# jhamrick/bayesian-quadrature

Hardware: AMD Instinct MI355X
Metric: bq_fit_posterior_throughput (higher is better)
Workload: dtype f64; 1 GPU; C2: d=1 N=1024 M=256 Gaussian integrand, w=dx, s=1e-3; curve_workload=C5 shard: 64 x (d=1 N=2048 M=256), w=dx, s=1e-2, on_curve=True, bordered_system=1344

## Files before the change

### bayesian-quadrature_amd/csrc/ctx.hip

```cpp
#include "host.h"

namespace bqh {

int prof_collect(bq_ctx *c)
{
    if (c->prof_events.empty())
        return BQ_OK;
    HIPCHK(c, hipStreamSynchronize(c->stream));
    if (c->aux)
        HIPCHK(c, hipStreamSynchronize(c->aux));
    if (c->prof_keep_timeline && !c->prof_origin)
        c->prof_origin = c->prof_events.front().a;
    for (auto &e : c->prof_events) {
        float ms = 0.f;
        if (hipEventElapsedTime(&ms, e.a, e.b) == hipSuccess) {
            c->prof_ms[e.cls] += ms;
            c->prof_n[e.cls] += 1;
            c->prof_work[e.cls] += e.work;
            if (c->prof_keep_timeline) {
                float t0 = 0.f;
                (void)hipEventElapsedTime(&t0, c->prof_origin, e.a);
                c->prof_timeline.insert(c->prof_timeline.end(),
                                        {(double)e.cls, (double)e.on_aux, (double)t0,
                                         (double)t0 + ms, e.work});
            }
        }
    }
    for (auto &e : c->prof_events) {
        if (e.a != c->prof_origin)
            (void)hipEventDestroy(e.a);
        (void)hipEventDestroy(e.b);
    }
    c->prof_events.clear();
    return BQ_OK;
}

int check_dims(bq_ctx *c, int64_t d, int64_t n)
{
    if (!c)
        return BQ_ERR_BAD_ARG;
    if (d < 1 || d > BQ_MAXD)
        return fail(c, BQ_ERR_BAD_ARG, "d must be in 1..%d", BQ_MAXD);
    if (n < 1 || n > (1 << 20))
        return fail(c, BQ_ERR_BAD_ARG, "n out of range");
    return BQ_OK;
}

int check_w(bq_ctx *c, int64_t d, double h, const double *w, double s)
{
    if (!w)
        return fail(c, BQ_ERR_BAD_ARG, "w is NULL");
    if (!(std::isfinite(h)) || !(std::isfinite(s)))
        return fail(c, BQ_ERR_BAD_ARG, "h and s must be finite");
    for (int k = 0; k < d; ++k)
        if (!(w[k] > 0.0) || !std::isfinite(w[k]))
            return fail(c, BQ_ERR_BAD_ARG, "w must be positive and finite");
    return BQ_OK;
}


}

using namespace bqh;

extern "C" int bq_device_count(int *count)
{
    if (!count)
        return BQ_ERR_BAD_ARG;
    int n = 0;
    if (hipGetDeviceCount(&n) != hipSuccess)
        n = 0;
    *count = n;
    return BQ_OK;
}

static int ctx_init(bq_ctx *c, int device)
{
    HIPCHK(c, hipSetDevice(device));
    c->device = device;
    hipDeviceProp_t prop;
    HIPCHK(c, hipGetDeviceProperties(&prop, device));
    c->cus = prop.multiProcessorCount > 0 ? prop.multiProcessorCount : 256;
    HIPCHK(c, hipEventCreate(&c->t0));
    HIPCHK(c, hipEventCreate(&c->t1));
    HIPCHK(c, hipEventCreateWithFlags(&c->ev_panel, hipEventDisableTiming));
    HIPCHK(c, hipEventCreateWithFlags(&c->ev_next, hipEventDisableTiming));
    HIPCHK(c, hipEventCreateWithFlags(&c->ev_fork, hipEventDisableTiming));
    HIPCHK(c, hipEventCreateWithFlags(&c->ev_top, hipEventDisableTiming));

    int lo = 0, hi = 0;
    HIPCHK(c, hipDeviceGetStreamPriorityRange(&lo, &hi));
    HIPCHK(c, hipStreamCreateWithPriority(&c->aux, hipStreamNonBlocking, hi));
    BQCHK(gemm_init(c));
    {
        void *h = nullptr;
        HIPCHK(c, hipHostMalloc(&h, 64, hipHostMallocMapped));
        c->flow_abort = static_cast<int *>(h);
        *c->flow_abort = 0;
    }
    static const struct {
        const char *name;
        int bq_ctx::*field;
    } switches[] = {
        {"BQ_TRSV_FLOW", &bq_ctx::trsv_flow},
        {"BQ_LOOKAHEAD", &bq_ctx::lookahead},
        {"BQ_DIAG_FIRST", &bq_ctx::diag_first},
        {"BQ_ASM_FUSE", &bq_ctx::asm_fuse},
        {"BQ_DF_SWEEP", &bq_ctx::df_sweep},
        {"BQ_DF_WG", &bq_ctx::df_wg},
        {"BQ_PAIR_BORDER", &bq_ctx::pair_border},
        {"BQ_DF_WG_ROWS", &bq_ctx::df_wg_rows},
        {"BQ_DF_EARLY", &bq_ctx::df_early},
        {"BQ_SOLVE_KCOPY", &bq_ctx::solve_kcopy},
        {"BQ_LA_MIN", &bq_ctx::la_min},
        {"BQ_GEMM_LDS", &bq_ctx::gemm_lds},
        {"BQ_FOLD_READOUT", &bq_ctx::fold_readout},
        {"BQ_POTF2_8W", &bq_ctx::potf2_8w},
        {"BQ_GEMM_KSPLIT", &bq_ctx::gemm_ksplit},
        {"BQ_GEMM_TILE", &bq_ctx::gemm_tile},
        {"BQ_GRAPH", &bq_ctx::use_graph},
    };
    for (const auto &sw : switches)
        if (const char *e = std::getenv(sw.name))
            c->*sw.field = std::atoi(e);
    return BQ_OK;
}

extern "C" int bq_ctx_create(int device, bq_ctx **out)
{
    if (!out)
        return BQ_ERR_BAD_ARG;
    *out = nullptr;
    bq_ctx *c = new (std::nothrow) bq_ctx();
    if (!c)
        return BQ_ERR_NOMEM;
    int st = ctx_init(c, device);
    if (st == BQ_OK) {
        hipError_t e = hipStreamCreateWithFlags(&c->stream, hipStreamNonBlocking);
        if (e != hipSuccess)
            st = fail(c, BQ_ERR_HIP, "hipStreamCreate: %s", hipGetErrorString(e));
        c->own_stream = true;
        c->cur = c->stream;
    }
    if (st != BQ_OK) {
        fprintf(stderr, "bq_ctx_create: %s\n", c->err);
        delete c;
        return st;
    }
    *out = c;
    return BQ_OK;
}

extern "C" int bq_ctx_create_on_stream(int device, void *hip_stream, bq_ctx **out)
{
    if (!out)
        return BQ_ERR_BAD_ARG;
    *out = nullptr;
    bq_ctx *c = new (std::nothrow) bq_ctx();
    if (!c)
        return BQ_ERR_NOMEM;
    int st = ctx_init(c, device);
    if (st != BQ_OK) {
        delete c;
        return st;
    }
    c->stream = static_cast<hipStream_t>(hip_stream);
    c->cur = c->stream;
    c->own_stream = false;
    *out = c;
    return BQ_OK;
}

extern "C" void bq_ctx_destroy(bq_ctx *c)
{
    if (!c)
        return;
    (void)hipSetDevice(c->device);
    (void)hipStreamSynchronize(c->stream);
    if (c->plan_cache) {
        bq_plan_destroy(c, c->plan_cache);
        c->plan_cache = nullptr;
    }
    for (auto &e : c->prof_events) {
        if (e.a != c->prof_origin)
            (void)hipEventDestroy(e.a);
        (void)hipEventDestroy(e.b);
    }
    if (c->prof_origin)
        (void)hipEventDestroy(c->prof_origin);
    if (c->t0)
        (void)hipEventDestroy(c->t0);
    if (c->t1)
        (void)hipEventDestroy(c->t1);
    if (c->hstage)
        (void)hipHostFree(c->hstage);
    c->hstage = nullptr;
    for (hipEvent_t e : {c->ev_panel, c->ev_next, c->ev_fork, c->ev_top})
        if (e)
            (void)hipEventDestroy(e);
    if (c->flow_abort)
        (void)hipHostFree(c->flow_abort);
    if (c->aux) {
        (void)hipStreamSynchronize(c->aux);
        (void)hipStreamDestroy(c->aux);
    }
    if (c->own_stream && c->stream)
        (void)hipStreamDestroy(c->stream);
    delete c;
}

extern "C" int bq_ctx_sync(bq_ctx *c)
{
    if (!c)
        return BQ_ERR_BAD_ARG;
    HIPCHK(c, hipSetDevice(c->device));
    HIPCHK(c, hipStreamSynchronize(c->stream));
    return flow_check(c);
}

extern "C" const char *bq_last_error(const bq_ctx *c) { return c ? c->err : "null context"; }

extern "C" int bq_device_info(bq_ctx *c, char *name, int *cus, size_t *hbm_bytes, int *clock_khz)
{
    if (!c)
        return BQ_ERR_BAD_ARG;
    hipDeviceProp_t prop;
    HIPCHK(c, hipGetDeviceProperties(&prop, c->device));
    if (name) {
        std::snprintf(name, 64, "%s (%s)", prop.name[0] ? prop.name : "AMD GPU", prop.gcnArchName);
    }
    if (cus)
        *cus = prop.multiProcessorCount;
    if (hbm_bytes)
        *hbm_bytes = prop.totalGlobalMem;
    if (clock_khz)
        *clock_khz = prop.clockRate;
    return BQ_OK;
}

extern "C" int bq_set_block(bq_ctx *c, int nb)
{
    if (!c || nb < 0 || (nb & 63))
        return c ? fail(c, BQ_ERR_BAD_ARG, "block must be a multiple of 64") : BQ_ERR_BAD_ARG;
    c->nb_override = nb;
    return BQ_OK;
}

extern "C" int bq_set_lookahead(bq_ctx *c, int on)
{
    if (!c)
        return BQ_ERR_BAD_ARG;
    c->lookahead = on ? 1 : 0;
    return BQ_OK;
}

extern "C" int bq_get_config(bq_ctx *c, int *nb, int *lookahead, int *min_rows)
{
    if (!c)
        return BQ_ERR_BAD_ARG;
    if (nb)
        *nb = c->nb_override;
    if (lookahead)
        *lookahead = c->lookahead;
    if (min_rows)
        *min_rows = c->la_min;
    return BQ_OK;
}

extern "C" int bq_ctx_stats(bq_ctx *c, int64_t *out, int n)
{
// ... 150 lines not shown
```

### bayesian-quadrature_amd/csrc/host.h

```cpp
#pragma once
#include <hip/hip_runtime.h>

#pragma GCC visibility push(default)
#include "../../include/bqhip.h"
#pragma GCC visibility pop

#include "types.h"

#include <algorithm>
#include <cmath>
#include <cstdarg>
#include <cstdio>
#include <cstdlib>
#include <cstring>
#include <limits>
#include <new>
#include <string>
#include <vector>

#define BQ_GUARD_BYTES 4096
inline bool &devbuf_guard()
{
    static bool on = std::getenv("BQ_GUARD") && std::atoi(std::getenv("BQ_GUARD"));
    return on;
}

struct DevBuf {
    void *p = nullptr;
    size_t bytes = 0;
    size_t guard = 0;
    DevBuf() = default;
    DevBuf(const DevBuf &) = delete;
    DevBuf &operator=(const DevBuf &) = delete;
    ~DevBuf() { release(); }
    void release()
    {
        if (p)
            (void)hipFree(p);
        p = nullptr;
        bytes = 0;
        guard = 0;
    }
    hipError_t alloc(size_t b)
    {
        release();
        if (b == 0)
            b = 8;
        const size_t g = devbuf_guard() ? BQ_GUARD_BYTES : 0;
        hipError_t e = hipMalloc(&p, b + g);
        if (e == hipSuccess && g)
            e = hipMemset(static_cast<char *>(p) + b, 0xA5, g);
        if (e == hipSuccess) {
            bytes = b;
            guard = g;
        } else {
            if (p)
                (void)hipFree(p);
            p = nullptr;
        }
        return e;
    }
    long guard_damage() const
    {
        if (!p || !guard)
            return 0;
        unsigned char h[BQ_GUARD_BYTES];
        if (hipMemcpy(h, static_cast<const char *>(p) + bytes, guard, hipMemcpyDeviceToHost) != hipSuccess)
            return -1;
        long bad = 0;
        for (size_t i = 0; i < guard; ++i)
            bad += h[i] != 0xA5;
        return bad;
    }
    double *d() const { return static_cast<double *>(p); }
    int *i() const { return static_cast<int *>(p); }
};

struct ProfEvent {
    hipEvent_t a, b;
    int cls;
    double work;
    int on_aux;
};

struct bq_ctx {
    int device = 0;
    hipStream_t stream = nullptr;
    hipStream_t aux = nullptr;
    hipStream_t cur = nullptr;
    hipEvent_t ev_panel = nullptr, ev_next = nullptr, ev_fork = nullptr, ev_top = nullptr;
    int lookahead = 1;
    int diag_first = 1;
    int df_sweep = 1;
    int df_wg = -1;
    int trsv_flow = 1;
    int *flow_abort = nullptr;
    long n_flow_fallback = 0;
    int pair_border = 1;
    int df_wg_rows = 1000;
    int df_early = 1;
    int solve_kcopy = 1;
    double *hstage = nullptr;
    size_t hstage_len = 0;
    int la_min = 3072;
    DevBuf panel_ws;
    DevBuf scratch;
    int gemm_lds = 1;
    int fold_readout = 1;
    int asm_fuse = 1;
    int potf2_8w = 1;
    int gemm_ksplit = 1;
    int gemm_tile = 0;
    int sharing = 0;
    int use_graph = 1;
    bool own_stream = false;
    int cus = 256;
    int nb_override = 0;
    bq_plan *plan_cache = nullptr;
    char err[512] = {0};
    hipEvent_t t0 = nullptr, t1 = nullptr;
    bool prof = false;
    std::vector<ProfEvent> prof_events;
    bool prof_keep_timeline = false;
    hipEvent_t prof_origin = nullptr;
    std::vector<double> prof_timeline;
    double prof_ms[BQ_K_NCLASS] = {0};
    int64_t prof_n[BQ_K_NCLASS] = {0};
    double prof_work[BQ_K_NCLASS] = {0};
    DevBuf gbuf;
    GaussParams gbuf_host{};
    bool gbuf_valid = false;
    DevBuf dinv64;
};

namespace bqh {

inline int fail(bq_ctx *c, int code, const char *fmt, ...)
{
    if (c) {
        va_list ap;
        va_start(ap, fmt);
        vsnprintf(c->err, sizeof c->err, fmt, ap);
        va_end(ap);
    }
    return code;
}

#define HIPCHK(c, call)                                                                        \
    do {                                                                                       \
        hipError_t e__ = (call);                                                               \
        if (e__ != hipSuccess)                                                                 \
            return bqh::fail((c), e__ == hipErrorOutOfMemory ? BQ_ERR_NOMEM : BQ_ERR_HIP,      \
                             "%s failed: %s (%s:%d)", #call, hipGetErrorString(e__), __FILE__, \
                             __LINE__);                                                        \
    } while (0)

#define BQCHK(call)                                                                            \
    do {                                                                                       \
        int s__ = (call);                                                                      \
        if (s__ != BQ_OK)                                                                      \
            return s__;                                                                        \
    } while (0)

inline long roundup(long v, long q) { return (v + q - 1) / q * q; }

inline unsigned long long launch_config_key(const bq_ctx *c)
{
    const int f[] = {c->nb_override, c->lookahead, c->la_min,   c->gemm_lds,  c->fold_readout,
                     c->potf2_8w,    c->gemm_ksplit, c->gemm_tile, c->diag_first, c->df_sweep,
                     c->df_wg,       c->df_early,   c->df_wg_rows};
    unsigned long long h = 1469598103934665603ull;
    for (int v : f)
        h = (h ^ (unsigned long long)(unsigned)v) * 1099511628211ull;
    return h;
}

inline long pick_ld(long ntot)
{
    long ld = ntot;
    if (ntot >= 1024 && (ntot % 512) == 0)
        ld += 64;
    return ld;
}

inline GaussParams make_params(int d, double h, const double *w, double s)
{
    GaussParams g;
    std::memset(&g, 0, sizeof g);
    double c = h * h;
    for (int k = 0; k < d; ++k) {
        c /= (std::sqrt(2.0 * M_PI) * w[k]);
        g.nh[k] = -0.5 / (w[k] * w[k]);
    }
    g.c = c;
    g.s2 = s * s;
    return g;
}

inline Layout make_layout(int n, int M, bool has_y)
{
    Layout L;
    L.n = n;
    L.npad = (int)roundup(n, 64);
    L.M = M;
    L.yrow = has_y ? L.npad + M : -1;
    L.ntot = (int)roundup(L.npad + M + (has_y ? 1 : 0), 64);
    return L;
}

struct Bracket {
    bq_ctx *c;
    ProfEvent ev;
    bool on;
    Bracket(bq_ctx *ctx, int cls, double work = 0.0) : c(ctx), on(ctx->prof)
    {
        if (on) {
            ev.cls = cls;
            ev.work = work;
            ev.on_aux = ctx->cur != ctx->stream;
            if (hipEventCreate(&ev.a) != hipSuccess || hipEventCreate(&ev.b) != hipSuccess) {
                on = false;
                return;
            }
            (void)hipEventRecord(ev.a, c->cur);
        }
    }
    ~Bracket()
    {
        if (on) {
            (void)hipEventRecord(ev.b, c->cur);
            c->prof_events.push_back(ev);
        }
    }
};

int prof_collect(bq_ctx *c);

struct Scratch {
    bq_ctx *c;
    size_t total = 0;
    explicit Scratch(bq_ctx *ctx) : c(ctx) {}
    size_t take(size_t doubles)
    {
        const size_t off = total;
        total += (doubles + 31) & ~(size_t)31;
        return off;
    }
    int commit()
    {
        if (c->scratch.bytes < total * sizeof(double)) {
            HIPCHK(c, hipStreamSynchronize(c->stream));
            HIPCHK(c, c->scratch.alloc(total * sizeof(double)));
        }
        return BQ_OK;
    }
    double *at(size_t off) const { return c->scratch.d() + off; }
};

int check_dims(bq_ctx *c, int64_t d, int64_t n);
int check_w(bq_ctx *c, int64_t d, double h, const double *w, double s);

int launch_gram_sym(bq_ctx *c, int d, const double *x, long xstride, const GaussParams *gp,
                    int gpstride, double *K, long ldk, long kstride, int n, int batch);
int launch_gram_cross(bq_ctx *c, int d, const double *x1, int n1, const double *x2, int n2,
                      const GaussParams &g, double *K, long ldk);
int launch_gram_cross_pad(bq_ctx *c, int d, const double *x1, int n1, int n1p, const double *x2,
                          int n2, int n2p, const GaussParams &g, double *K, long ldk);

struct FirstStep {
    double *S0 = nullptr;
    long lds = 0, sstride = 0;
    double *dinv = nullptr;
    int *info = nullptr;
    double *scal = nullptr;
};
int launch_assemble(bq_ctx *c, int d, const double *pts, long pstride, const double *y,
                    long ystride, const GaussParams *gp, int gpstride, double *A, long lda,
                    long astride, Layout L, int batch, const FirstStep &fs = FirstStep(),
                    int jcols = 0);
int launch_assemble_region(bq_ctx *c, const GramSeed &sd, double *A, long lda, long astride, int m,
                           int n, int batch);
int launch_potf2(bq_ctx *c, double *A, long lda, long astride, int j0, double *dinv, long dstride,
                 int *info, int batch);
int launch_potrf_wg(bq_ctx *c, double *A, long lda, long astride, int kb, double *rec, long rstride,
                    int *info, int col0, int batch);
int launch_trsm_blk(bq_ctx *c, double *X, long ldx, long xstride, int m, const double *L11,
                    long ldl, long lstride, const double *dinv, long dstride, int batch);
int launch_diag_winv(bq_ctx *c, const double *L, long ldl, int npad, double *dw);
int launch_panel_step(bq_ctx *c, double *A, long lda, long astride, int batch, int nrb,
                      double *Sin, double *Sout, long lds, long sstride, int K0, int j0,
                      double *dinv_in, double *dinv_out, int has_next, int first, double *SL,
                      int *info, double work);
int launch_slab_first(bq_ctx *c, double *A, long lda, long astride, int batch, double *S, long lds,
                      long sstride, int ntot, double *dinv, int *info, int col0,
                      long dstride = BQ_DINV_STRIDE);
int launch_slab_step(bq_ctx *c, double *A, long lda, long astride, int batch, double *Sin,
                     double *Sout, long lds, long sstride, int ntot, int j0, double *dinv_in,
                     double *dinv_out, int fnext, int last, int *info, int col0,
                     const SlabOut &out, long long *stamps, double work,
                     long dstride = BQ_DINV_STRIDE);

int gemm_init(bq_ctx *c);
bool gemm_uses_lds(const bq_ctx *c, int m, int n, int k, int lower, int batch);
size_t grad_parts(int npad, int d);
int launch_logml_grad(bq_ctx *c, int d, const double *Y, int npad, const GradJob &gj,
                      const GradScale &sc, double *grad);
int launch_gemm(bq_ctx *c, int cls, double *C, long ldc, long cstride, const double *P, long ldp,
                long pstride, const double *Q, long qsj, long qsk, long qstride, int m, int n,
                int k, int lower, int batch, int fuse_j0 = -1, double *dinv = nullptr,
                long dstride = 0, int *info = nullptr, int ccut = 0,
                const GramSeed *seed = nullptr);
bool gemm_trsm_ok(const bq_ctx *c, int m, int n, int k);
int launch_gemm_trsm(bq_ctx *c, double *C, long ldc, long cstride, const double *P, long ldp,
                     long pstride, const double *Q, long ldq, long qstride, int m, int n, int k,
                     const double *Lss, long ldl, long lstride, const double *wrec, long wstride,
                     int batch);
int launch_trsm_sweep(bq_ctx *c, double *X, long ldx, long xstride, int m, const double *L11,
                      long ldl, long lstride, const double *rec, long rstride, int kb, int batch);
int launch_gemm_rows(bq_ctx *c, int cls, double *C, long ldc, const double *P, long ldp,
                     const double *Q, long qsj, long qsk, int m, int n, int k);
int launch_rows_step(bq_ctx *c, int mrows, const RowsJob &a, const RowsJob &b, double work);
int launch_rows_fused(bq_ctx *c, int mrows, const RowsJob &a, double *C, long ldc, const double *P,
                      long ldp, const double *Q, long ldq, int n, int k, bool qt, double work);
// ... 261 lines not shown
```

### bayesian-quadrature_amd/csrc/k_panel.hip

```cpp
#include "host.h"
#include "gram.h"
#include "trsm.h"
#include "slab.h"

namespace bqh {

template <int D>
void launch_assemble_d(bq_ctx *c, const double *pts, long pstride, const double *y, long ystride,
                       const GaussParams *gp, int gpstride, double *A, long lda, long astride,
                       Layout L, int batch, const FirstStep &fs, int jcols)
{
    dim3 grid((L.ntot + 127) / 128, ((jcols > 0 ? jcols : L.ntot) + 63) / 64, batch);
    const long wgs = (long)grid.x * grid.y * grid.z;
    if (fs.S0 && c->potf2_8w && wgs <= 2L * c->cus)
        hipLaunchKernelGGL((assemble_first_kernel<D, 8>), grid, dim3(512), 0, c->cur, pts, pstride, y,
                           ystride, gp, gpstride, A, lda, astride, L, fs.S0, fs.lds, fs.sstride,
                           fs.dinv, (long)BQ_DINV_STRIDE, fs.info, fs.scal);
    else if (fs.S0)
        hipLaunchKernelGGL((assemble_first_kernel<D, 4>), grid, dim3(256), 0, c->cur, pts, pstride, y,
                           ystride, gp, gpstride, A, lda, astride, L, fs.S0, fs.lds, fs.sstride,
                           fs.dinv, (long)BQ_DINV_STRIDE, fs.info, fs.scal);
    else
        hipLaunchKernelGGL(assemble_kernel<D>, grid, dim3(256), 0, c->cur, pts, pstride, y, ystride,
                           gp, gpstride, A, lda, astride, L);
}

int launch_assemble(bq_ctx *c, int d, const double *pts, long pstride, const double *y,
                    long ystride, const GaussParams *gp, int gpstride, double *A, long lda,
                    long astride, Layout L, int batch, const FirstStep &fs, int jcols)
{
    if (jcols < 0 || (jcols & 63) || jcols > L.ntot || (jcols > 0 && fs.S0))
        return fail(c, BQ_ERR_BAD_ARG, "assemble: column limit");
    const double cols = jcols > 0 ? jcols : L.ntot;
    Bracket br(c, BQ_K_GRAM, 8.0 * cols * (L.ntot - 0.5 * cols + 0.5) * batch);
    switch (d) {
    case 1: launch_assemble_d<1>(c, pts, pstride, y, ystride, gp, gpstride, A, lda, astride, L, batch, fs, jcols); break;
    case 2: launch_assemble_d<2>(c, pts, pstride, y, ystride, gp, gpstride, A, lda, astride, L, batch, fs, jcols); break;
    case 3: launch_assemble_d<3>(c, pts, pstride, y, ystride, gp, gpstride, A, lda, astride, L, batch, fs, jcols); break;
    case 4: launch_assemble_d<4>(c, pts, pstride, y, ystride, gp, gpstride, A, lda, astride, L, batch, fs, jcols); break;
    case 5: launch_assemble_d<5>(c, pts, pstride, y, ystride, gp, gpstride, A, lda, astride, L, batch, fs, jcols); break;
    case 6: launch_assemble_d<6>(c, pts, pstride, y, ystride, gp, gpstride, A, lda, astride, L, batch, fs, jcols); break;
    case 7: launch_assemble_d<7>(c, pts, pstride, y, ystride, gp, gpstride, A, lda, astride, L, batch, fs, jcols); break;
    case 8: launch_assemble_d<8>(c, pts, pstride, y, ystride, gp, gpstride, A, lda, astride, L, batch, fs, jcols); break;
    default: return fail(c, BQ_ERR_BAD_ARG, "d must be in 1..%d", BQ_MAXD);
    }
    HIPCHK(c, hipGetLastError());
    return BQ_OK;
}

int launch_assemble_region(bq_ctx *c, const GramSeed &sd, double *A, long lda, long astride, int m,
                           int n, int batch)
{
    if (m <= 0 || n <= 0)
        return BQ_OK;
    if ((m & 63) || (n & 63) || (sd.r & 63) || (sd.c & 63))
        return fail(c, BQ_ERR_BAD_ARG, "assemble_region: multiples of 64");
    Bracket br(c, BQ_K_GRAM, 8.0 * m * n * batch);
    const dim3 grid((m + 127) / 128, n / 64, batch);
#define BQ_ASM_REGION(D_)                                                                          \
    case D_:                                                                                       \
        hipLaunchKernelGGL(assemble_region_kernel<D_>, grid, dim3(256), 0, c->cur, sd.pts,         \
                           sd.pstride, sd.y, sd.ystride, sd.gp, sd.gpstride, A, lda, astride, sd.L, \
                           sd.r, sd.c, m, n);                                                      \
        break;
    switch (sd.d) {
        BQ_ASM_REGION(1)
        BQ_ASM_REGION(2)
        BQ_ASM_REGION(3)
        BQ_ASM_REGION(4)
        BQ_ASM_REGION(5)
        BQ_ASM_REGION(6)
        BQ_ASM_REGION(7)
        BQ_ASM_REGION(8)
    default:
        return fail(c, BQ_ERR_BAD_ARG, "d must be in 1..%d", BQ_MAXD);
    }
#undef BQ_ASM_REGION
    HIPCHK(c, hipGetLastError());
    return BQ_OK;
}

int launch_potf2(bq_ctx *c, double *A, long lda, long astride, int j0, double *dinv, long dstride,
                 int *info, int batch)
{
    Bracket br(c, BQ_K_POTF2, 64.0 * 64 * 64 / 3.0 * batch);
    if (c->potf2_8w && batch <= c->cus)
        hipLaunchKernelGGL(potf2_kernel<8>, dim3(1, 1, batch), dim3(512), 0, c->cur, A, lda, astride,
                           j0, dinv, dstride, info);
    else
        hipLaunchKernelGGL(potf2_kernel<4>, dim3(1, 1, batch), dim3(256), 0, c->cur, A, lda, astride,
                           j0, dinv, dstride, info);
    HIPCHK(c, hipGetLastError());
    return BQ_OK;
}

int launch_potrf_wg(bq_ctx *c, double *A, long lda, long astride, int kb, double *rec, long rstride,
                    int *info, int col0, int batch)
{
    Bracket br(c, BQ_K_POTF2, (double)kb * kb * kb / 3.0 * batch);
    hipLaunchKernelGGL(potrf_wg_kernel, dim3(batch), dim3(512), 0, c->cur, A, lda, astride, kb, rec,
                       rstride, info, col0);
    HIPCHK(c, hipGetLastError());
    return BQ_OK;
}

int launch_trsm_blk(bq_ctx *c, double *X, long ldx, long xstride, int m, const double *L11,
                    long ldl, long lstride, const double *dinv, long dstride, int batch)
{
    if (m <= 0)
        return BQ_OK;
    Bracket br(c, BQ_K_TRSM, 64.0 * 64 * (double)m * batch);
    hipLaunchKernelGGL(trsm_blk_kernel, dim3((m + 63) / 64, 1, batch), dim3(256), 0, c->cur, X, ldx,
                       xstride, m, L11, ldl, lstride, dinv, dstride);
    HIPCHK(c, hipGetLastError());
    return BQ_OK;
}

int launch_diag_winv(bq_ctx *c, const double *L, long ldl, int npad, double *dw)
{
    hipLaunchKernelGGL(diag_winv_kernel, dim3(npad / 64), dim3(256), 0, c->stream, L, ldl, dw);
    HIPCHK(c, hipGetLastError());
    return BQ_OK;
}

int launch_panel_step(bq_ctx *c, double *A, long lda, long astride, int batch, int nrb,
                      double *Sin, double *Sout, long lds, long sstride, int K0, int j0,
                      double *dinv_in, double *dinv_out, int has_next, int first, double *SL,
                      int *info, double work)
{
    Bracket br(c, BQ_K_GEMM, work);
    hipLaunchKernelGGL(panel_step_kernel, dim3(nrb, 1, batch), dim3(256), 0, c->cur, A, lda,
                       astride, Sin, Sout, lds, sstride, K0, j0, dinv_in, dinv_out,
                       (long)BQ_DINV_STRIDE, has_next, first, SL, info);
    HIPCHK(c, hipGetLastError());
    return BQ_OK;
}

int launch_slab_first(bq_ctx *c, double *A, long lda, long astride, int batch, double *S, long lds,
                      long sstride, int ntot, double *dinv, int *info, int col0, long dstride)
{
    Bracket br(c, BQ_K_POTF2, 64.0 * 64 * 64 / 3.0 * batch);
    hipLaunchKernelGGL(slab_first_kernel, dim3(ntot / 64, 1, batch), dim3(256), 0, c->cur, A, lda,
                       astride, S, lds, sstride, ntot, dinv, dstride, info, col0);
    HIPCHK(c, hipGetLastError());
    return BQ_OK;
}

int launch_slab_step(bq_ctx *c, double *A, long lda, long astride, int batch, double *Sin,
                     double *Sout, long lds, long sstride, int ntot, int j0, double *dinv_in,
                     double *dinv_out, int fnext, int last, int *info, int col0,
                     const SlabOut &out, long long *stamps, double work, long dstride)
{
    const int T = (ntot - j0 - 64) / 64;
    Bracket br(c, BQ_K_SYRK_SMALL, work);
    const long wgs = (long)T * (T + 1) / 2 * batch;
    const bool w8 = c->potf2_8w && fnext && wgs <= c->cus;
    if (stamps && w8)
        hipLaunchKernelGGL((slab_step_kernel<true, 8>), dim3(T * (T + 1) / 2, 1, batch), dim3(512), 0,
                           c->cur, A, lda, astride, Sin, Sout, lds, sstride, ntot, j0, dinv_in,
                           dinv_out, dstride, fnext, last, info, col0, stamps, out);
    else if (stamps)
        hipLaunchKernelGGL((slab_step_kernel<true, 4>), dim3(T * (T + 1) / 2, 1, batch), dim3(256), 0,
                           c->cur, A, lda, astride, Sin, Sout, lds, sstride, ntot, j0, dinv_in,
                           dinv_out, dstride, fnext, last, info, col0, stamps, out);
    else if (w8)
        hipLaunchKernelGGL((slab_step_kernel<false, 8>), dim3(T * (T + 1) / 2, 1, batch), dim3(512),
                           0, c->cur, A, lda, astride, Sin, Sout, lds, sstride, ntot, j0, dinv_in,
                           dinv_out, dstride, fnext, last, info, col0,
                           (long long *)nullptr, out);
    else
        hipLaunchKernelGGL((slab_step_kernel<false, 4>), dim3(T * (T + 1) / 2, 1, batch), dim3(256),
                           0, c->cur, A, lda, astride, Sin, Sout, lds, sstride, ntot, j0, dinv_in,
                           dinv_out, dstride, fnext, last, info, col0,
                           (long long *)nullptr, out);
    HIPCHK(c, hipGetLastError());
    return BQ_OK;
}

}
```

### bayesian-quadrature_amd/csrc/slab.h

```cpp
#pragma once
#include "common.h"
#include "potf2.h"


__device__ __forceinline__ void slab_load16(const double *__restrict__ S, long lds,
                                            double (&t)[4][4])
{
#pragma unroll
    for (int c = 0; c < 4; ++c)
#pragma unroll
        for (int r = 0; r < 4; ++r)
            t[c][r] = S[(long)(16 * c + 4 * r) * lds];
}

__device__ __forceinline__ void slab_solve16(const double (&t)[4][4], const double (&la)[4][3][4],
                                             const double (&wneg)[4][4], double4_t (&x)[4])
{
#pragma unroll
    for (int c = 0; c < 4; ++c) {
        double4_t acc = {-t[c][0], -t[c][1], -t[c][2], -t[c][3]};
#pragma unroll
        for (int bb = 0; bb < c; ++bb)
#pragma unroll
            for (int r = 0; r < 4; ++r)
                acc = __builtin_amdgcn_mfma_f64_16x16x4f64(la[c][bb][r], x[bb][r], acc, 0, 0, 0);
        double4_t xc = {0.0, 0.0, 0.0, 0.0};
#pragma unroll
        for (int r = 0; r < 4; ++r)
            xc = __builtin_amdgcn_mfma_f64_16x16x4f64(wneg[c][r], acc[r], xc, 0, 0, 0);
        x[c] = xc;
    }
}

#define BQ_SLAB_FW (10 * 256)
#define DIAG_NB(w) ((w) < 2 ? 3 : 2)
#define DIAG_RB(w, s) ((w) == 0 ? ((s) > 0 ? 1 : 0) : ((w) == 1 ? 2 : 3))
#define DIAG_CB(w, s) ((w) == 0 ? ((s) == 2 ? 1 : 0) : (((w) == 3 ? 2 : 0) + ((w) >= 2 && (s) == 2 ? 1 : (s))))

template <bool STAMP, int NW = 4>
__global__ __launch_bounds__(64 * NW, NW == 4 ? 2 : 1) void slab_step_kernel(double *__restrict__ A, long lda,
                                                        long astride,
                                                        const double *__restrict__ Sin,
                                                        double *__restrict__ Sout, long lds,
                                                        long sstride, int ntot, int j0,
                                                        const double *__restrict__ din,
                                                        double *__restrict__ dout, long dstride,
                                                        int factor_next, int last,
                                                        int *__restrict__ info, int col0,
                                                        long long *stamps, SlabOut out)
{
#define BQ_SSTAMP(k, dep)                                                                          \
    if (STAMP) {                                                                                   \
        asm volatile("" ::"v"(dep));                                                               \
        __builtin_amdgcn_sched_barrier(0);                                                         \
        if (blockIdx.x == 0 && blockIdx.z == 0 && threadIdx.x == 0)                                \
            stamps[k] = (long long)__builtin_amdgcn_s_memtime();                                   \
        __builtin_amdgcn_sched_barrier(0);                                                         \
    }
    BQ_SSTAMP(0, 0)
    __shared__ __attribute__((aligned(16))) double plds[4096 + BQ_SLAB_FW];
    double *const Qs = plds;
    double *const Ts = plds;
    __builtin_amdgcn_s_setprio(3);
    const int b = blockIdx.z;
    const int lane = threadIdx.x & 63;
    const int wave = __builtin_amdgcn_readfirstlane(threadIdx.x >> 6);
    int bx, by;
    tri_decode(blockIdx.x, bx, by);
    A += (long)b * astride;
    Sin += (long)b * sstride;
    Sout += (long)b * sstride;
    din += (long)b * dstride;
    dout += (long)b * dstride;
    const int r0 = j0 + 64;
    const int Rb = r0 + 64 * bx, Cb = r0 + 64 * by;
    const int l15 = lane & 15, l4 = lane >> 4;
    if (NW == 8 && wave >= 4) {
        __syncthreads();
        __syncthreads();
        if (blockIdx.x == 0 && factor_next) {
            __syncthreads();
            __syncthreads();
            potf2_body<8>(A + r0 + (long)r0 * lda, lda, col0 + r0, dout, info + b, plds, Ts, 64,
                          (long long *)nullptr, out.scal ? out.scal + 4 * b + 1 : nullptr);
        }
        return;
    }

    double la[4][3][4], wneg[4][4], tp[4][4], tq[4][4];
    double4_t acc[4];
    {
        double *Fs = plds + 4096;
        double *Ws = plds + 4096 + 6 * 256;
        {
            const int t = threadIdx.x, ti = t & 15, tk = t >> 4;
            const double *L11 = A + j0 + (long)j0 * lda + ti + (long)tk * lda;
            double f[6], wv[4];
#pragma unroll
            for (int c = 1; c < 4; ++c)
#pragma unroll
                for (int bb = 0; bb < c; ++bb)
                    f[(c * (c - 1)) / 2 + bb] = L11[16 * c + (long)(16 * bb) * lda];
#pragma unroll
            for (int q = 0; q < 4; ++q)
                wv[q] = din[64 + 256 * q + t];
            if (bx != by)
                slab_load16(Sin + Cb + 16 * wave + l15 + (long)l4 * lds, lds, tq);
            slab_load16(Sin + Rb + 16 * wave + l15 + (long)l4 * lds, lds, tp);
            if (bx == by) {
                acc[2] = double4_t{0.0, 0.0, 0.0, 0.0};
#pragma unroll
                for (int sb = 0; sb < 3; ++sb)
                    if (sb < DIAG_NB(wave)) {
                        const double *Cin = A + Rb + 16 * DIAG_RB(wave, sb) + l15 +
                                            (long)(Cb + 16 * DIAG_CB(wave, sb) + l4) * lda;
#pragma unroll
                        for (int r = 0; r < 4; ++r)
                            acc[sb][r] = -Cin[(long)(4 * r) * lda];
                    }
            } else {
                const double *Cin = A + Rb + 16 * wave + l15 + (long)(Cb + l4) * lda;
#pragma unroll
                for (int cb = 0; cb < 4; ++cb)
#pragma unroll
                    for (int r = 0; r < 4; ++r)
                        acc[cb][r] = -Cin[(long)(16 * cb + 4 * r) * lda];
            }
#pragma unroll
            for (int q = 0; q < 6; ++q)
                Fs[256 * q + t] = f[q];
#pragma unroll
            for (int q = 0; q < 4; ++q)
                Ws[256 * q + t] = -wv[q];
        }
        __syncthreads();
#pragma unroll
        for (int c = 0; c < 4; ++c)
#pragma unroll
            for (int r = 0; r < 4; ++r)
                wneg[c][r] = Ws[256 * c + 64 * r + l15 + 16 * l4];
#pragma unroll
        for (int c = 1; c < 4; ++c)
#pragma unroll
            for (int bb = 0; bb < c; ++bb)
#pragma unroll
                for (int r = 0; r < 4; ++r)
                    la[c][bb][r] = Fs[256 * ((c * (c - 1)) / 2 + bb) + l15 + 16 * (l4 + 4 * r)];
    }
    BQ_SSTAMP(1, la[3][2][3] + wneg[3][3])
    double4_t xp[4];
    if (bx != by) {
        double4_t xq[4];
        slab_solve16(tq, la, wneg, xq);
#pragma unroll
        for (int c = 0; c < 4; ++c)
#pragma unroll
            for (int r = 0; r < 4; ++r)
                Qs[(16 * c + l4 + 4 * r) * 64 + 16 * wave + l15] = xq[c][r];
    }
    slab_solve16(tp, la, wneg, xp);
    if (bx == by) {
#pragma unroll
        for (int c = 0; c < 4; ++c)
#pragma unroll
            for (int r = 0; r < 4; ++r)
                Qs[(16 * c + l4 + 4 * r) * 64 + 16 * wave + l15] = xp[c][r];
    }
    BQ_SSTAMP(2, xp[3][3])
    if (by == 0) {
        double *Lw = A + Rb + 16 * wave + l15 + (long)(j0 + l4) * lda;
#pragma unroll
        for (int c = 0; c < 4; ++c)
#pragma unroll
            for (int r = 0; r < 4; ++r)
                Lw[(long)(16 * c + 4 * r) * lda] = xp[c][r];
    }
    __syncthreads();
    BQ_SSTAMP(3, acc[1][3] + acc[0][0])
    if (bx == by) {
        const int rb0 = DIAG_RB(wave, 0), rb1 = DIAG_RB(wave, 1), rb2 = DIAG_RB(wave, 2);
        const int cb0 = DIAG_CB(wave, 0), cb1 = DIAG_CB(wave, 1), cb2 = DIAG_CB(wave, 2);
#pragma unroll
        for (int c = 0; c < 4; ++c)
#pragma unroll
            for (int r = 0; r < 4; ++r) {
                const double *qrow = Qs + (16 * c + l4 + 4 * r) * 64 + l15;
                acc[0] = __builtin_amdgcn_mfma_f64_16x16x4f64(qrow[16 * cb0], qrow[16 * rb0], acc[0],
                                                              0, 0, 0);
                acc[1] = __builtin_amdgcn_mfma_f64_16x16x4f64(qrow[16 * cb1], qrow[16 * rb1], acc[1],
                                                              0, 0, 0);
                acc[2] = __builtin_amdgcn_mfma_f64_16x16x4f64(qrow[16 * cb2], qrow[16 * rb2],
                                                              acc[2], 0, 0, 0);
            }
    } else {
#pragma unroll
        for (int c = 0; c < 4; ++c)
#pragma unroll
            for (int r = 0; r < 4; ++r) {
                const double pf = xp[c][r];
                const double *qrow = Qs + (16 * c + l4 + 4 * r) * 64 + l15;
#pragma unroll
                for (int cb = 0; cb < 4; ++cb)
                    acc[cb] =
                        __builtin_amdgcn_mfma_f64_16x16x4f64(qrow[16 * cb], pf, acc[cb], 0, 0, 0);
            }
    }
    BQ_SSTAMP(4, acc[1][3] + acc[0][0])
    if (blockIdx.x == 0 && factor_next) {
        __syncthreads();
#pragma unroll
        for (int sb = 0; sb < 3; ++sb)
            if (sb < DIAG_NB(wave)) {
#pragma unroll
                for (int r = 0; r < 4; ++r)
                    Ts[16 * DIAG_RB(wave, sb) + l15 +
                       64 * (16 * DIAG_CB(wave, sb) + l4 + 4 * r)] = -acc[sb][r];
            }
        __syncthreads();
        potf2_body<NW>(A + r0 + (long)r0 * lda, lda, col0 + r0, dout, info + b, plds, Ts, 64,
                       (STAMP && blockIdx.z == 0) ? stamps + 5 : nullptr,
                       out.scal ? out.scal + 4 * b + 1 : nullptr);
        return;
    }
    const bool to_s = by == 0 && bx > 0 && !last;
    double *Cout = to_s ? Sout + Rb + 16 * wave + l15 + (long)l4 * lds
                        : A + Rb + 16 * wave + l15 + (long)(Cb + l4) * lda;
    const long ldo = to_s ? lds : lda;
#define BQ_SLAB_EMIT(ROW_, COL_, S_)                                                               \
    {                                                                                              \
        const int row_ = (ROW_), col_ = (COL_);                                                    \
        const double s_ = (S_);                                                                    \
        if (row_ == col_ && row_ >= out.npad && row_ < out.npad + out.M && out.var)                \
            out.var[(long)b * out.mstride + (row_ - out.npad)] = s_;                               \
        if (row_ == out.yrow) {                                                                    \
            if (col_ >= out.npad && col_ < out.npad + out.M && out.mean)                           \
                out.mean[(long)b * out.mstride + (col_ - out.npad)] = -s_;                         \
            if (col_ == out.yrow) {                                                                \
                const double qf_ = -s_, ld_ = out.scal[4 * b + 1];                                 \
                out.scal[4 * b + 2] = qf_;                                                         \
                out.scal[4 * b + 0] =                                                              \
                    -0.5 * qf_ - 0.5 * ld_ - 0.5 * (double)out.n * 1.8378770664093453;             \
            }                                                                                      \
        }                                                                                          \
    }
    const bool emit = last && out.scal != nullptr;
    if (bx == by) {
#pragma unroll
        for (int sb = 0; sb < 3; ++sb)
            if (sb < DIAG_NB(wave)) {
                double *Cd = A + Rb + 16 * DIAG_RB(wave, sb) + l15 +
                             (long)(Cb + 16 * DIAG_CB(wave, sb) + l4) * lda;
#pragma unroll
                for (int r = 0; r < 4; ++r)
                    Cd[(long)(4 * r) * lda] = -acc[sb][r];
                if (emit) {
#pragma unroll
                    for (int r = 0; r < 4; ++r)
                        BQ_SLAB_EMIT(Rb + 16 * DIAG_RB(wave, sb) + l15,
                                     Cb + 16 * DIAG_CB(wave, sb) + l4 + 4 * r, -acc[sb][r])
                }
            }
    } else {
#pragma unroll
        for (int cb = 0; cb < 4; ++cb)
#pragma unroll
            for (int r = 0; r < 4; ++r)
                Cout[(long)(16 * cb + 4 * r) * ldo] = -acc[cb][r];
        if (emit) {
#pragma unroll
            for (int cb = 0; cb < 4; ++cb)
#pragma unroll
                for (int r = 0; r < 4; ++r)
                    BQ_SLAB_EMIT(Rb + 16 * wave + l15, Cb + 16 * cb + l4 + 4 * r, -acc[cb][r])
        }
    }
#undef BQ_SLAB_EMIT
#undef BQ_SSTAMP
}

template <int D, int NW = 4>
__global__ __launch_bounds__(64 * NW) void assemble_first_kernel(
    const double *__restrict__ pts, long pstride, const double *__restrict__ y, long ystride,
    const GaussParams *__restrict__ gp, int gpstride, double *__restrict__ A, long lda,
    long astride, Layout L, double *__restrict__ S0, long lds, long sstride,
    double *__restrict__ dinv, long dstride, int *__restrict__ info, double *__restrict__ scal)
{
    __shared__ __attribute__((aligned(16))) double plds[BQ_POTF2_LDS_DOUBLES];
    const int b = blockIdx.z;
    A += (long)b * astride;
    if (NW == 4 || threadIdx.x < 256)
        assemble_tile<D>(pts + (long)b * pstride, y + (long)b * ystride, gp[(long)b * gpstride],
                         A, lda, L, S0 + (long)b * sstride, lds);
    if (blockIdx.x == 0 && blockIdx.y == 0) {
        if (threadIdx.x == 0) {
            info[b] = 0;
            if (scal)
                scal[4 * b + 1] = 0.0;
        }
        asm volatile("s_waitcnt vmcnt(0)" ::: "memory");
        __syncthreads();
        __builtin_amdgcn_s_setprio(3);
        potf2_body<NW>(A, lda, 0, dinv + (long)b * dstride, info + b, plds, nullptr, 0, nullptr,
                       scal ? scal + 4 * b + 1 : nullptr, L.n);
    }
}

__global__ __launch_bounds__(256) void slab_first_kernel(double *__restrict__ A, long lda,
                                                         long astride, double *__restrict__ S,
                                                         long lds, long sstride, int ntot,
                                                         double *__restrict__ dinv, long dstride,
                                                         int *__restrict__ info, int col0)
{
    __shared__ __attribute__((aligned(16))) double plds[BQ_POTF2_LDS_DOUBLES];
    const int b = blockIdx.z;
    A += (long)b * astride;
    if (blockIdx.x == 0) {
        __builtin_amdgcn_s_setprio(3);
        potf2_body(A, lda, col0, dinv + (long)b * dstride, info + b, plds);
        return;
    }
    const int i = 64 * (int)blockIdx.x + (threadIdx.x & 63);
    const int jb = (threadIdx.x >> 6) * 16;
    if (i < ntot) {
        double *dst = S + (long)b * sstride + i + (long)jb * lds;
        const double *src = A + i + (long)jb * lda;
#pragma unroll
        for (int j = 0; j < 16; ++j)
            dst[(long)j * lds] = src[(long)j * lda];
    }
}

__global__ __launch_bounds__(256) void panel_step_kernel(double *__restrict__ A, long lda,
                                                         long astride,
                                                         const double *__restrict__ Sin,
                                                         double *__restrict__ Sout, long lds,
                                                         long sstride, int K0, int j0,
                                                         const double *__restrict__ din,
                                                         double *__restrict__ dout, long dstride,
                                                         int has_next, int first,
                                                         double *__restrict__ SL,
                                                         int *__restrict__ info)
{
    __shared__ __attribute__((aligned(16))) double plds[BQ_POTF2_LDS_DOUBLES];
    double *const Qs = plds;
    double *const Ts = plds;
    __builtin_amdgcn_s_setprio(3);
    const int b = blockIdx.z;
    const int lane = threadIdx.x & 63;
    const int wave = __builtin_amdgcn_readfirstlane(threadIdx.x >> 6);
    A += (long)b * astride;
    Sin += (long)b * sstride;
    Sout += (long)b * sstride;
    din += (long)b * dstride;
    dout += (long)b * dstride;
    const int r0 = j0 + 64;
    const int Rb = r0 + 64 * blockIdx.x;
    const int l15 = lane & 15, l4 = lane >> 4;
    SL += (long)b * 4096;
    const double *Sp = first ? A + (long)j0 * lda : Sin;
    const long ldsp = first ? lda : lds;
    if (!first && j0 - K0 == 64 && blockIdx.x == 0) {
        double *dst = A + j0 + (long)(j0 - 64) * lda;
        for (int e = threadIdx.x; e < 4096; e += 256)
            dst[(e & 63) + (long)(e >> 6) * lda] = SL[e];
    }

    double la[4][3][4], wneg[4][4];
    {
        const double *L11 = A + j0 + (long)j0 * lda + l15 + (long)l4 * lda;
        const double *W = din + 64 + l15 + 16 * l4;
#pragma unroll
        for (int c = 0; c < 4; ++c)
#pragma unroll
            for (int r = 0; r < 4; ++r)
                wneg[c][r] = -W[256 * c + 64 * r];
#pragma unroll
        for (int c = 1; c < 4; ++c)
#pragma unroll
            for (int bb = 0; bb < c; ++bb)
#pragma unroll
                for (int r = 0; r < 4; ++r)
                    la[c][bb][r] = L11[16 * c + (long)(16 * bb + 4 * r) * lda];
    }
    double4_t xp[4];
    if (has_next && blockIdx.x != 0) {
        double4_t xq[4];
        double tq[4][4];
        slab_load16(Sp + r0 + 16 * wave + l15 + (long)l4 * ldsp, ldsp, tq);
        slab_solve16(tq, la, wneg, xq);
#pragma unroll
        for (int c = 0; c < 4; ++c)
#pragma unroll
            for (int r = 0; r < 4; ++r)
                Qs[(16 * c + l4 + 4 * r) * 64 + 16 * wave + l15] = xq[c][r];
    }
    {
        double tp[4][4];
        slab_load16(Sp + Rb + 16 * wave + l15 + (long)l4 * ldsp, ldsp, tp);
        slab_solve16(tp, la, wneg, xp);
    }
    {
        const bool side = first && has_next && blockIdx.x == 0 && gridDim.x > 1;
        double *Lw = side ? SL + 16 * wave + l15 + 64 * l4
                          : A + Rb + 16 * wave + l15 + (long)(j0 + l4) * lda;
        const long ldw = side ? 64 : lda;
#pragma unroll
        for (int c = 0; c < 4; ++c)
#pragma unroll
            for (int r = 0; r < 4; ++r)
                Lw[(long)(16 * c + 4 * r) * ldw] = xp[c][r];
    }
    if (!has_next)
        return;
    if (blockIdx.x == 0) {
#pragma unroll
        for (int c = 0; c < 4; ++c)
#pragma unroll
            for (int r = 0; r < 4; ++r)
                Qs[(16 * c + l4 + 4 * r) * 64 + 16 * wave + l15] = xp[c][r];
    }
    const double *Cin = A + Rb + 16 * wave + l15 + (long)(r0 + l4) * lda;
    double4_t acc[4];
#pragma unroll
    for (int cb = 0; cb < 4; ++cb)
#pragma unroll
        for (int r = 0; r < 4; ++r)
            acc[cb][r] = -Cin[(long)(16 * cb + 4 * r) * lda];
    {
        const double *Pg = A + Rb + 16 * wave + l15 + (long)(K0 + l4) * lda;
        const double *Qg = A + r0 + l15 + (long)(K0 + l4) * lda;
        const int kend = j0 - K0;
        double pa[4], qa[4][4], pb[4], qb[4][4];
#define BQ_PANEL_LOAD(PF, QF, KK)                                                                  \
    _Pragma("unroll") for (int t = 0; t < 4; ++t)                                                  \
    {                                                                                              \
        PF[t] = Pg[(long)((KK) + 4 * t) * lda];                                                    \
        _Pragma("unroll") for (int cb = 0; cb < 4; ++cb) QF[t][cb] =                               \
            Qg[16 * cb + (long)((KK) + 4 * t) * lda];                                              \
    }
#define BQ_PANEL_MFMA(PF, QF)                                                                      \
    _Pragma("unroll") for (int t = 0; t < 4; ++t) _Pragma("unroll") for (int cb = 0; cb < 4; ++cb) \
        acc[cb] = __builtin_amdgcn_mfma_f64_16x16x4f64(QF[t][cb], PF[t], acc[cb], 0, 0, 0);
        if (kend > 0) {
            BQ_PANEL_LOAD(pa, qa, 0)
            for (int kk = 0; kk < kend; kk += 32) {
                BQ_PANEL_LOAD(pb, qb, kk + 16)
                __builtin_amdgcn_sched_barrier(0);
                BQ_PANEL_MFMA(pa, qa)
                __builtin_amdgcn_sched_barrier(0);
                const int kn = kk + 32 < kend ? kk + 32 : kk;
                BQ_PANEL_LOAD(pa, qa, kn)
                __builtin_amdgcn_sched_barrier(0);
                BQ_PANEL_MFMA(pb, qb)
                __builtin_amdgcn_sched_barrier(0);
            }
        }
#undef BQ_PANEL_LOAD
#undef BQ_PANEL_MFMA
    }
    __syncthreads();
#pragma unroll
    for (int c = 0; c < 4; ++c)
#pragma unroll
        for (int r = 0; r < 4; ++r) {
            const double pf = xp[c][r];
            const double *qrow = Qs + (16 * c + l4 + 4 * r) * 64 + l15;
#pragma unroll
            for (int cb = 0; cb < 4; ++cb)
                acc[cb] = __builtin_amdgcn_mfma_f64_16x16x4f64(qrow[16 * cb], pf, acc[cb], 0, 0, 0);
        }
    if (blockIdx.x == 0) {
        __syncthreads();
#pragma unroll
        for (int cb = 0; cb < 4; ++cb)
#pragma unroll
            for (int r = 0; r < 4; ++r)
                Ts[16 * wave + l15 + 64 * (16 * cb + l4 + 4 * r)] = -acc[cb][r];
        __syncthreads();
        potf2_body(A + r0 + (long)r0 * lda, lda, r0, dout, info + b, plds, Ts, 64);
        return;
    }
    double *Cout = Sout + Rb + 16 * wave + l15 + (long)l4 * lds;
#pragma unroll
    for (int cb = 0; cb < 4; ++cb)
#pragma unroll
        for (int r = 0; r < 4; ++r)
            Cout[(long)(16 * cb + 4 * r) * lds] = -acc[cb][r];
}

__device__ __forceinline__ void wg_update32(double *__restrict__ C, long ldc,
                                            const double *__restrict__ P,
                                            const double *__restrict__ Q, long ldp, int row0,
                                            int col0, int lane)
{
    const int l15 = lane & 15, l4 = lane >> 4;
    double pa[16][2], qa[16][2], cold[2][2][4];
#pragma unroll
    for (int h = 0; h < 2; ++h) {
        const double *pp = P + row0 + 16 * h + l15 + (long)l4 * ldp;
        const double *qq = Q + col0 + 16 * h + l15 + (long)l4 * ldp;
#pragma unroll
        for (int ks = 0; ks < 16; ++ks) {
            pa[ks][h] = pp[(long)(4 * ks) * ldp];
            qa[ks][h] = qq[(long)(4 * ks) * ldp];
        }
    }
#pragma unroll
    for (int tm = 0; tm < 2; ++tm)
#pragma unroll
        for (int tn = 0; tn < 2; ++tn)
#pragma unroll
            for (int rr = 0; rr < 4; ++rr)
                cold[tm][tn][rr] =
                    C[(row0 + 16 * tm + l15) + (long)(col0 + 16 * tn + l4 + 4 * rr) * ldc];
    __builtin_amdgcn_sched_barrier(0);
    double4_t acc[2][2];
#pragma unroll
    for (int tm = 0; tm < 2; ++tm)
#pragma unroll
        for (int tn = 0; tn < 2; ++tn)
            acc[tm][tn] = (double4_t){0.0, 0.0, 0.0, 0.0};
#pragma unroll
    for (int ks = 0; ks < 16; ++ks)
#pragma unroll
        for (int tm = 0; tm < 2; ++tm)
#pragma unroll
            for (int tn = 0; tn < 2; ++tn)
                acc[tm][tn] =
                    __builtin_amdgcn_mfma_f64_16x16x4f64(qa[ks][tn], pa[ks][tm], acc[tm][tn], 0, 0, 0);
#pragma unroll
    for (int tm = 0; tm < 2; ++tm)
#pragma unroll
        for (int tn = 0; tn < 2; ++tn) {
            if (col0 + 16 * tn >= row0 + 16 * tm + 16)
                continue;
#pragma unroll
            for (int rr = 0; rr < 4; ++rr)
                C[(row0 + 16 * tm + l15) + (long)(col0 + 16 * tn + l4 + 4 * rr) * ldc] =
                    cold[tm][tn][rr] - acc[tm][tn][rr];
        }
}

__global__ __launch_bounds__(512) void potrf_wg_kernel(double *__restrict__ A, long lda,
                                                       long astride, int kb,
                                                       double *__restrict__ rec, long rstride,
                                                       int *__restrict__ info, int col0)
{
    __shared__ __attribute__((aligned(16))) double plds[BQ_POTF2_LDS_DOUBLES];
    __builtin_amdgcn_s_setprio(3);
    const int b = blockIdx.x;
    A += (long)b * astride;
    rec += (long)b * rstride;
    const int lane = threadIdx.x & 63;
    const int wave = __builtin_amdgcn_readfirstlane(threadIdx.x >> 6);
    const int l15 = lane & 15, l4 = lane >> 4;
    const int ns = kb >> 6;
    for (int s = 0; s < ns; ++s) {
        double *Ass = A + 64 * s + (long)(64 * s) * lda;
        double *rs = rec + (long)s * BQ_DINV_HALF;
        potf2_body<8>(Ass, lda, col0 + 64 * s, rs, info + b, plds);
        asm volatile("s_waitcnt vmcnt(0)" ::: "memory");
        __syncthreads();
        const int nr = ns - s - 1;
        if (nr == 0)
            break;
        const int r0 = 64 * (s + 1);
        {
            double la[4][3][4], wneg[4][4];
            const double *L11 = Ass + l15 + (long)l4 * lda;
            const double *W = rs + 64 + l15 + 16 * l4;
#pragma unroll
            for (int c = 0; c < 4; ++c)
#pragma unroll
                for (int r = 0; r < 4; ++r)
                    wneg[c][r] = -W[256 * c + 64 * r];
#pragma unroll
            for (int c = 1; c < 4; ++c)
#pragma unroll
                for (int bb = 0; bb < c; ++bb)
#pragma unroll
                    for (int r = 0; r < 4; ++r)
                        la[c][bb][r] = L11[16 * c + (long)(16 * bb + 4 * r) * lda];
            for (int task = wave; task < 4 * nr; task += 8) {
                double *Xr = A + r0 + 16 * task + l15 + (long)(64 * s + l4) * lda;
                double t[4][4];
                double4_t x[4];
                slab_load16(Xr, lda, t);
                slab_solve16(t, la, wneg, x);
#pragma unroll
                for (int c = 0; c < 4; ++c)
#pragma unroll
                    for (int r = 0; r < 4; ++r)
                        Xr[(long)(16 * c + 4 * r) * lda] = x[c][r];
            }
        }
        asm volatile("s_waitcnt vmcnt(0)" ::: "memory");
        __syncthreads();
        {
            const double *Pn = A + r0 + (long)(64 * s) * lda;
            double *Cn = A + r0 + (long)r0 * lda;
            const int ntask = 4 * (nr * (nr + 1) / 2);
            for (int task = wave; task < ntask; task += 8) {
                int ti, tj;
                tri_decode(task >> 2, ti, tj);
                const int q = task & 3;
                const int row0 = 64 * ti + 32 * (q & 1), cl0 = 64 * tj + 32 * (q >> 1);
                if (cl0 > row0)
                    continue;
                wg_update32(Cn, lda, Pn, Pn, lda, row0, cl0, lane);
            }
        }
        asm volatile("s_waitcnt vmcnt(0)" ::: "memory");
        __syncthreads();
    }
}
```

Measured before the change: 3949 problems/s.

## Use 8-wave workgroups in panel and slab steps to split Q-solve across waves

Adds an 8-wave variant of the panel step kernel in which waves 4-7 solve the Q slab (or run the potf2 of the next diagonal block) while waves 0-3 solve the P slab. In the slab step's 8-wave path, the off-diagonal Q solve also moves to the upper waves, with the fragment setup factored into a helper. The 8-wave slab path now applies up to a configurable multiple of CU count, effectively always by default. The goal is more latency hiding and parallelism in the small-batch triangular update. The cost is extra barriers, higher register and LDS pressure, and some risk of barrier-count mismatches between waves.

```diff
diff --git a/bayesian-quadrature_amd/csrc/ctx.hip b/bayesian-quadrature_amd/csrc/ctx.hip
--- a/bayesian-quadrature_amd/csrc/ctx.hip
+++ b/bayesian-quadrature_amd/csrc/ctx.hip
@@ -116,6 +116,7 @@
         {"BQ_GEMM_LDS", &bq_ctx::gemm_lds},
         {"BQ_FOLD_READOUT", &bq_ctx::fold_readout},
         {"BQ_POTF2_8W", &bq_ctx::potf2_8w},
+        {"BQ_SLAB8_ROUNDS", &bq_ctx::slab8_rounds},
         {"BQ_GEMM_KSPLIT", &bq_ctx::gemm_ksplit},
         {"BQ_GEMM_TILE", &bq_ctx::gemm_tile},
         {"BQ_GRAPH", &bq_ctx::use_graph},
diff --git a/bayesian-quadrature_amd/csrc/host.h b/bayesian-quadrature_amd/csrc/host.h
--- a/bayesian-quadrature_amd/csrc/host.h
+++ b/bayesian-quadrature_amd/csrc/host.h
@@ -109,6 +109,7 @@
     int fold_readout = 1;
     int asm_fuse = 1;
     int potf2_8w = 1;
+    int slab8_rounds = 1 << 20;
     int gemm_ksplit = 1;
     int gemm_tile = 0;
     int sharing = 0;
@@ -168,7 +169,7 @@
 {
     const int f[] = {c->nb_override, c->lookahead, c->la_min,   c->gemm_lds,  c->fold_readout,
                      c->potf2_8w,    c->gemm_ksplit, c->gemm_tile, c->diag_first, c->df_sweep,
-                     c->df_wg,       c->df_early,   c->df_wg_rows};
+                     c->df_wg,       c->df_early,   c->df_wg_rows, c->slab8_rounds};
     unsigned long long h = 1469598103934665603ull;
     for (int v : f)
         h = (h ^ (unsigned long long)(unsigned)v) * 1099511628211ull;
diff --git a/bayesian-quadrature_amd/csrc/k_panel.hip b/bayesian-quadrature_amd/csrc/k_panel.hip
--- a/bayesian-quadrature_amd/csrc/k_panel.hip
+++ b/bayesian-quadrature_amd/csrc/k_panel.hip
@@ -129,9 +129,15 @@
                       int *info, double work)
 {
     Bracket br(c, BQ_K_GEMM, work);
-    hipLaunchKernelGGL(panel_step_kernel, dim3(nrb, 1, batch), dim3(256), 0, c->cur, A, lda,
-                       astride, Sin, Sout, lds, sstride, K0, j0, dinv_in, dinv_out,
-                       (long)BQ_DINV_STRIDE, has_next, first, SL, info);
+    const bool beside_bulk = c->sharing != 0 && (long)nrb * batch > 64;
+    if (c->potf2_8w && !beside_bulk && (long)nrb * batch <= c->cus)
+        hipLaunchKernelGGL(panel_step_kernel<8>, dim3(nrb, 1, batch), dim3(512), 0, c->cur, A, lda,
+                           astride, Sin, Sout, lds, sstride, K0, j0, dinv_in, dinv_out,
+                           (long)BQ_DINV_STRIDE, has_next, first, SL, info);
+    else
+        hipLaunchKernelGGL(panel_step_kernel<4>, dim3(nrb, 1, batch), dim3(256), 0, c->cur, A, lda,
+                           astride, Sin, Sout, lds, sstride, K0, j0, dinv_in, dinv_out,
+                           (long)BQ_DINV_STRIDE, has_next, first, SL, info);
     HIPCHK(c, hipGetLastError());
     return BQ_OK;
 }
@@ -146,6 +152,11 @@
     return BQ_OK;
 }
 
+static long slab8_limit(const bq_ctx *c)
+{
+    return (long)(c->slab8_rounds > 1 ? c->slab8_rounds : 1) * c->cus;
+}
+
 int launch_slab_step(bq_ctx *c, double *A, long lda, long astride, int batch, double *Sin,
                      double *Sout, long lds, long sstride, int ntot, int j0, double *dinv_in,
                      double *dinv_out, int fnext, int last, int *info, int col0,
@@ -154,7 +165,7 @@
     const int T = (ntot - j0 - 64) / 64;
     Bracket br(c, BQ_K_SYRK_SMALL, work);
     const long wgs = (long)T * (T + 1) / 2 * batch;
-    const bool w8 = c->potf2_8w && fnext && wgs <= c->cus;
+    const bool w8 = c->potf2_8w && fnext && wgs <= slab8_limit(c);
     if (stamps && w8)
         hipLaunchKernelGGL((slab_step_kernel<true, 8>), dim3(T * (T + 1) / 2, 1, batch), dim3(512), 0,
                            c->cur, A, lda, astride, Sin, Sout, lds, sstride, ntot, j0, dinv_in,
diff --git a/bayesian-quadrature_amd/csrc/slab.h b/bayesian-quadrature_amd/csrc/slab.h
--- a/bayesian-quadrature_amd/csrc/slab.h
+++ b/bayesian-quadrature_amd/csrc/slab.h
@@ -30,6 +30,24 @@
             xc = __builtin_amdgcn_mfma_f64_16x16x4f64(wneg[c][r], acc[r], xc, 0, 0, 0);
         x[c] = xc;
     }
+}
+
+__device__ __forceinline__ void slab_frags(const double *Fs, int l15, int l4, double (&la)[4][3][4],
+                                           double (&wneg)[4][4])
+{
+    const double *Ws = Fs + 6 * 256;
+#pragma unroll
+    for (int c = 0; c < 4; ++c)
+#pragma unroll
+        for (int r = 0; r < 4; ++r)
+            wneg[c][r] = Ws[256 * c + 64 * r + l15 + 16 * l4];
+#pragma unroll
+    for (int c = 1; c < 4; ++c)
+#pragma unroll
+        for (int bb = 0; bb < c; ++bb)
+#pragma unroll
+            for (int r = 0; r < 4; ++r)
+                la[c][bb][r] = Fs[256 * ((c * (c - 1)) / 2 + bb) + l15 + 16 * (l4 + 4 * r)];
 }
 
 #define BQ_SLAB_FW (10 * 256)
@@ -76,6 +94,23 @@
     const int Rb = r0 + 64 * bx, Cb = r0 + 64 * by;
     const int l15 = lane & 15, l4 = lane >> 4;
     if (NW == 8 && wave >= 4) {
+        if (bx != by) {
+            const int wq = wave - 4;
+            double tq[4][4];
+            slab_load16(Sin + Cb + 16 * wq + l15 + (long)l4 * lds, lds, tq);
+            __syncthreads();
+            double la[4][3][4], wneg[4][4];
+            slab_frags(plds + 4096, l15, l4, la, wneg);
+            double4_t xq[4];
+            slab_solve16(tq, la, wneg, xq);
+#pragma unroll
+            for (int c = 0; c < 4; ++c)
+#pragma unroll
+                for (int r = 0; r < 4; ++r)
+                    Qs[(16 * c + l4 + 4 * r) * 64 + 16 * wq + l15] = xq[c][r];
+            __syncthreads();
+            return;
+        }
         __syncthreads();
         __syncthreads();
         if (blockIdx.x == 0 && factor_next) {
@@ -104,7 +139,7 @@
 #pragma unroll
             for (int q = 0; q < 4; ++q)
                 wv[q] = din[64 + 256 * q + t];
-            if (bx != by)
+            if (NW == 4 && bx != by)
                 slab_load16(Sin + Cb + 16 * wave + l15 + (long)l4 * lds, lds, tq);
             slab_load16(Sin + Rb + 16 * wave + l15 + (long)l4 * lds, lds, tp);
             if (bx == by) {
@@ -134,22 +169,11 @@
                 Ws[256 * q + t] = -wv[q];
         }
         __syncthreads();
-#pragma unroll
-        for (int c = 0; c < 4; ++c)
-#pragma unroll
-            for (int r = 0; r < 4; ++r)
-                wneg[c][r] = Ws[256 * c + 64 * r + l15 + 16 * l4];
-#pragma unroll
-        for (int c = 1; c < 4; ++c)
-#pragma unroll
-            for (int bb = 0; bb < c; ++bb)
-#pragma unroll
-                for (int r = 0; r < 4; ++r)
-                    la[c][bb][r] = Fs[256 * ((c * (c - 1)) / 2 + bb) + l15 + 16 * (l4 + 4 * r)];
+        slab_frags(Fs, l15, l4, la, wneg);
     }
     BQ_SSTAMP(1, la[3][2][3] + wneg[3][3])
     double4_t xp[4];
-    if (bx != by) {
+    if (NW == 4 && bx != by) {
         double4_t xq[4];
         slab_solve16(tq, la, wneg, xq);
 #pragma unroll
@@ -330,7 +354,8 @@
     }
 }
 
-__global__ __launch_bounds__(256) void panel_step_kernel(double *__restrict__ A, long lda,
+template <int NW = 4>
+__global__ __launch_bounds__(64 * NW) void panel_step_kernel(double *__restrict__ A, long lda,
                                                          long astride,
                                                          const double *__restrict__ Sin,
                                                          double *__restrict__ Sout, long lds,
@@ -361,8 +386,17 @@
     const long ldsp = first ? lda : lds;
     if (!first && j0 - K0 == 64 && blockIdx.x == 0) {
         double *dst = A + j0 + (long)(j0 - 64) * lda;
-        for (int e = threadIdx.x; e < 4096; e += 256)
+        for (int e = threadIdx.x; e < 4096; e += 64 * NW)
             dst[(e & 63) + (long)(e >> 6) * lda] = SL[e];
+    }
+    if (NW == 8 && wave >= 4 && (!has_next || blockIdx.x == 0)) {
+        if (!has_next)
+            return;
+        __syncthreads();
+        __syncthreads();
+        __syncthreads();
+        potf2_body<8>(A + r0 + (long)r0 * lda, lda, r0, dout, info + b, plds, Ts, 64);
+        return;
     }
 
     double la[4][3][4], wneg[4][4];
@@ -383,16 +417,21 @@
                     la[c][bb][r] = L11[16 * c + (long)(16 * bb + 4 * r) * lda];
     }
     double4_t xp[4];
-    if (has_next && blockIdx.x != 0) {
+    if (has_next && blockIdx.x != 0 && (NW == 4 || wave >= 4)) {
+        const int wq = wave & 3;
         double4_t xq[4];
         double tq[4][4];
-        slab_load16(Sp + r0 + 16 * wave + l15 + (long)l4 * ldsp, ldsp, tq);
+        slab_load16(Sp + r0 + 16 * wq + l15 + (long)l4 * ldsp, ldsp, tq);
         slab_solve16(tq, la, wneg, xq);
 #pragma unroll
         for (int c = 0; c < 4; ++c)
 #pragma unroll
             for (int r = 0; r < 4; ++r)
-                Qs[(16 * c + l4 + 4 * r) * 64 + 16 * wave + l15] = xq[c][r];
+                Qs[(16 * c + l4 + 4 * r) * 64 + 16 * wq + l15] = xq[c][r];
+        if (NW == 8) {
+            __syncthreads();
+            return;
+        }
     }
     {
         double tp[4][4];
@@ -477,7 +516,7 @@
             for (int r = 0; r < 4; ++r)
                 Ts[16 * wave + l15 + 64 * (16 * cb + l4 + 4 * r)] = -acc[cb][r];
         __syncthreads();
-        potf2_body(A + r0 + (long)r0 * lda, lda, r0, dout, info + b, plds, Ts, 64);
+        potf2_body<NW>(A + r0 + (long)r0 * lda, lda, r0, dout, info + b, plds, Ts, 64);
         return;
     }
     double *Cout = Sout + Rb + 16 * wave + l15 + (long)l4 * lds;
```

Result: faster. 4005 problems/s (median of 6 runs) (+1.4%).
